# marcinmiklitz/pywindow

Hardware: AMD Instinct MI355X
Metric: trajectory frames/sec full_analysis (pore+windows), CC3 1k-frame (higher is better)
Workload: dtype f64

## Files before the change

pywindow_amd/csrc/pw_unit.hpp:

```cpp
#pragma once
#include "../../include/pywindow_amd.h"
#include "pw_lbfgsb.hpp"
#include "pw_math.hpp"
#include "pw_team.hpp"
#include <string.h>

#if defined(PW_PROFILE) && defined(__HIPCC__)
__shared__ unsigned long long pw_prof_lds[32];
#define PW_PROF_BASE(ws) ((unsigned long long*)pw_prof_lds)
#endif
#if defined(PW_PROFILE) && defined(__HIP_DEVICE_COMPILE__)
#define PW_T0(var) long long var = wall_clock64()
#if defined(PW_ZPROF) && defined(PW_LB_FINE)
#define PW_T1(ws, slot, var) do { (void)var; } while (0)
#elif defined(PW_BARRIER_PROF)
#define PW_T1(ws, slot, var) do { (void)var; if (T::lane() == 0) { unsigned long long w_ = 0; \
        for (int k_ = 0; k_ < T::NWAVES; ++k_) w_ += atomicExch(&pw_bar_acc[k_], 0ull); \
        atomicAdd(&pw_prof_lds[slot], w_); } } while (0)
#else
#define PW_T1(ws, slot, var) do { if (T::lane() == 0) atomicAdd(&pw_prof_lds[slot], (unsigned long long)(wall_clock64() - var)); } while (0)
#endif
#else
#define PW_T0(var) do {} while (0)
#define PW_T1(ws, slot, var) do {} while (0)
#endif

namespace pw {

constexpr double GOLDEN_ANGLE = 2.399963229728653;
constexpr double FOUR_PI = 12.566370614359172;
constexpr double FOUR_THIRDS_PI = 4.1887902047863905;
constexpr double TWO_PI = 6.283185307179586;
constexpr double ONE_PI = 3.141592653589793;

constexpr int PW_KCLS = 8;
constexpr double PW_PATH_POINTS_MAX = 1048576.0;
struct ClassInfo {
    int k;
    int off[PW_KCLS + 1];
    double vdw[PW_KCLS];
};
struct Frame {
    ldouble *x, *y, *z, *xx;
    const ldouble* vdw;
    const lint* perm;
    const PW_LDS ClassInfo* cls;
};

struct TeamWorkspace {
    double* knn;
    double* pts;
    double* vals;
    int* surv_k;
    int* labels;
    unsigned char* flag;
    unsigned long long* adj;
    double* xw;
    int* xw_ok;
    int p_cap;
    const unsigned* nb_off;
    const unsigned short* nb_idx;
    const double* nb_unit;
    const double* nb_bound;
    pw_extra_window* xwin;
    unsigned* xwin_count;
    unsigned xwin_cap;
    double leaf[256];
    double acc8[8 * 160];
    int leaf_tab[324];
    unsigned long long prof[32];
    const unsigned* rsq;
    pw_unit_debug* dbg_base;
    long unit;
};
PW_HD inline size_t team_slab_bytes(int p_cap) { return (size_t)p_cap * 192; }
PW_HD inline size_t team_adj_words(int p_cap) { return (size_t)p_cap * (size_t)(p_cap / 64); }
PW_HD inline int round_p_cap(long p) {
    if (p < PW_P_MAX) p = PW_P_MAX;
    return (int)((p + 127) & ~127l);
}
PW_HD inline int params_p_cap(double adjust_windows, double adjust_average) {
    double a = adjust_windows > adjust_average ? adjust_windows : adjust_average;
    if (!(a > 0.0)) a = 1.0;
    double want = 2100.0 * a;
    if (want > 4.0e6) want = 4.0e6;
    return round_p_cap((long)want + 1);
}
PW_HD inline void bind_team_slab(TeamWorkspace* ws, unsigned char* slab, int p_cap) {
    const size_t p = (size_t)p_cap;
    double* d = (double*)slab;
    ws->knn = d; d += 10 * p;
    ws->pts = d; d += 3 * p;
    ws->vals = d; d += p;
    ws->xw = d; d += 7 * p;
    int* i = (int*)d;
    ws->surv_k = i; i += p;
    ws->labels = i; i += p;
    ws->xw_ok = i; i += p;
    ws->flag = (unsigned char*)i;
    ws->p_cap = p_cap;
}

struct UnitVars {
    double com[3];
    double mw;
    int mw_given;
    double centroid[3];
    double maxd;
    int maxd_i, maxd_j;
    double pore_g;
    int pore_atom;
    double opt_c[3];
    double opt_g;
    int opt_atom;
    double shift[3];
    ClassInfo cls;
    int cls_cnt[PW_KCLS];
    double eps;
// ... 1329 lines not shown
        k0 += NP;
    };
    while (k0 <= chunks && ok) {
        if (chunks - k0 + 1 <= 5) tile(std::integral_constant<int, 5>());
        else tile(std::integral_constant<int, 6>());
    }
    if (n_eval) *n_eval += chunks + 1;
    if (!ok) return false;
    *out_2gap = best * 2.0;
    *out_pos = pos;
    out_chunk[0] = cx; out_chunk[1] = cy; out_chunk[2] = cz;
    return true;
}

struct PathSteps {
    double cx, cy, cz, cd, rinv;
    int chunks;
    bool bracket;
};
PW_HD inline PathSteps path_steps(const Frame& F, double vx, double vy, double vz, double inc, double xx_max) {
    PathSteps s;
    const double nrm = norm3(vx, vy, vz);
    const double fd = np_floordiv(nrm, inc);
    s.bracket = F.cls->k > 0 && fd >= 1.0 && fd <= PW_PATH_POINTS_MAX && nrm < PW_INF;
    s.chunks = s.bracket ? (int)fd : 0;
    s.cd = (double)s.chunks;
    s.cx = vx / s.cd; s.cy = vy / s.cd; s.cz = vz / s.cd;
    const double cc = sq3(s.cx, s.cy, s.cz);
    s.rinv = 1.0 / cc;
    const double bound = (64.0 * 0x1p-53) * (xx_max + sq3(vx, vy, vz));
    s.bracket = s.bracket && cc > 0.0 && cc < PW_INF && s.rinv < PW_INF && bound < PW_INF && cc * (1.0 - 1e-6) > bound;
    return s;
}
PW_NOINLINE PW_HD inline bool path_bracket_thread(const Frame& F, int n, double cx, double cy, double cz, int chunks,
                                                  double rinv, double m0, double* out_2gap, int* n_eval,
                                                  const lint* cand = nullptr, const lint* coff = nullptr,
                                                  long* n_terms = nullptr) {
    (void)n;
    const auto& C = *F.cls;
    const double cd = (double)chunks;
    double best = PW_INF;
    long terms = 0;
    for (int g = 0; g < C.k; ++g) {
        double m2 = PW_INF;
        auto atom = [&](double x, double y, double z, double xx) __attribute__((always_inline)) {
            const double t = pw_fma(z, cz, pw_fma(x, cx, y * cy)) * rinv;
            const double lo = __builtin_fmin(__builtin_fmax(__builtin_floor(t), 1.0), cd);
            const double hi = __builtin_fmin(lo + 1.0, cd);
            const double ax = cx * lo, ay = cy * lo, az = cz * lo;
            const double bx = cx * hi, by = cy * hi, bz = cz * hi;
            const double ga = pw_fma(z, az, pw_fma(x, ax, y * ay));
            const double gb = pw_fma(z, bz, pw_fma(x, bx, y * by));
            const double va = pw_m2add(ga, xx) + sq3(ax, ay, az);
            const double vb = pw_m2add(gb, xx) + sq3(bx, by, bz);
            m2 = __builtin_fmin(m2, __builtin_fmin(va, vb));
        };
        auto span = [&](int c, const int chi, auto at) __attribute__((always_inline)) {
            terms += 2 * (chi - c);
            for (; c + 4 <= chi; c += 4) {
                int i[4];
                double x[4], y[4], z[4], xx[4];
#pragma unroll
                for (int j = 0; j < 4; ++j) i[j] = at(c + j);
#pragma unroll
                for (int j = 0; j < 4; ++j) { x[j] = F.x[i[j]]; y[j] = F.y[i[j]]; z[j] = F.z[i[j]]; xx[j] = F.xx[i[j]]; }
#pragma unroll
                for (int j = 0; j < 4; ++j) atom(x[j], y[j], z[j], xx[j]);
            }
            for (; c < chi; ++c) {
                const int i = at(c);
                atom(F.x[i], F.y[i], F.z[i], F.xx[i]);
            }
        };
        if (cand) span(coff[g], coff[g + 1], [&](int c) __attribute__((always_inline)) { return (int)cand[c]; });
        else span(C.off[g], C.off[g + 1], [](int c) __attribute__((always_inline)) { return c; });
        const double d = pw_sqrt(m2 > 0.0 ? m2 : 0.0);
        best = __builtin_fmin(best, d - C.vdw[g]);
    }
    if (n_eval) *n_eval += chunks + 1;
    if (n_terms) *n_terms += terms;
    if (!(m0 > 0.0) || !(best > 0.0)) return false;
    *out_2gap = (best < m0 ? best : m0) * 2.0;
    return true;
}

template <class T>
PW_HD inline bool wave_path_candidates(const Frame& F, int n, bool have, double vx, double vy, double vz, double inc,
                                       double m0, lint* cand, lint* coff) {
    const auto& C = *F.cls;
    if (C.k == 0 || !(m0 > 0.0)) return false;
    double uz_lo = PW_INF, uz_hi = -PW_INF, t1 = PW_INF;
    bool odd = false;
    if (have) {
        const double nrm = norm3(vx, vy, vz);
        odd = !(nrm >= inc * (1.0 + 1e-9)) || !(nrm < PW_INF) || !(inc > 0.0);
        if (!odd) uz_lo = uz_hi = vz / nrm;
    }
    if (T::wave_any(odd)) return false;
    double z1 = T::wave_min(uz_lo) - 1e-9, z2 = -T::wave_min(-uz_hi) + 1e-9;
    t1 = inc * (1.0 - 1e-9);
    if (!(z1 <= z2)) return false;
    z1 = pw_max(z1, -1.0); z2 = pw_min(z2, 1.0);
    const double s1 = pw_sqrt(pw_max(1.0 - z1 * z1, 0.0)), s2 = pw_sqrt(pw_max(1.0 - z2 * z2, 0.0));
    const double m0p = m0 * (1.0 + 1e-9) + 1e-9;
    const int mycut = T::lane() <= C.k ? C.off[T::lane() <= PW_KCLS ? T::lane() : PW_KCLS] : n;
    int mycount = 0, cnt = 0;
    for (int base = 0; base < n; base += T::WSIZE) {
        const int i = base + T::lane();
        bool keep = false;
        if (i < n) {
            const double xx = F.xx[i], z = F.z[i], r = F.vdw[i];
            const double rho = pw_sqrt(xx);
            const double zd = rho > 0.0 ? z / rho : 0.0;
            const double sd = pw_sqrt(pw_max(1.0 - zd * zd, 0.0));
            double c1 = 1.0;
            if (zd > z2) c1 = sd * s2 + zd * z2;
            else if (zd < z1) c1 = sd * s1 + zd * z1;
            c1 = pw_min(1.0, pw_max(0.0, c1 + 1e-9));
            const double ts = rho * c1;
            const double low = ts >= t1 ? xx * (1.0 - c1 * c1) : (xx + t1 * t1) - 2.0 * t1 * ts;
            const double lim = (r + m0p) * (r + m0p);
            keep = !(low * (1.0 - 1e-9) - 1e-9 > lim * (1.0 + 1e-9));
        }
        const unsigned long long bal = T::ballot(keep);
        const int pos = cnt + __builtin_popcountll(bal & ((1ull << T::lane()) - 1ull));
        if (keep) cand[pos] = i;
        if (T::WSIZE > 1) {
            int w = mycut - base;
            w = w < 0 ? 0 : (w > 64 ? 64 : w);
            mycount += __builtin_popcountll(bal & (w >= 64 ? ~0ull : ((1ull << w) - 1ull)));
        }
        cnt += __builtin_popcountll(bal);
    }
    if (T::WSIZE > 1) {
        if (T::lane() <= C.k) coff[T::lane()] = mycount;
    } else {
        int c = 0;
        for (int g = 0; g <= C.k; ++g) {
            while (c < cnt && cand[c] < C.off[g]) ++c;
            coff[g] = c;
        }
    }
    T::wave_sync();
    return true;
}

PW_HD inline size_t template_groups_bytes(int n) {
    const size_t npad = (size_t)((n + 1) & ~1);
    return ((sizeof(ClassInfo) + 7) & ~(size_t)7) + npad * 4 * 2 + npad * 8 + 8;
}
PW_HD inline double molecular_weight_sum(const double* mass, int n) {
    double tot = 0.0;
    for (int s0 = 0; s0 < n; s0 += 8192) {
        double part = np_sum_lean(mass + s0, n - s0 < 8192 ? n - s0 : 8192);
        tot = s0 == 0 ? part : tot + part;
    }
    return tot;
}
inline void template_groups_build(const double* vdw, const double* mass, int n, unsigned char* blob) {
    const size_t npad = (size_t)((n + 1) & ~1);
    ClassInfo* cls = (ClassInfo*)blob;
    int* inv = (int*)(blob + ((sizeof(ClassInfo) + 7) & ~(size_t)7));
    int* perm = inv + npad;
    double* vs = (double*)(perm + npad);
    memset(blob, 0, template_groups_bytes(n));
    int ngrp = 0;
// ... 1034 lines not shown
#pragma unroll
        for (int g = 0; g <= PW_KCLS; ++g) {
            const int first = g < kk ? T::uniform_i(C->off[g]) : n;
            const int below = first - 64 * t;
            const unsigned long long lt = below >= 64 ? ~0ull : (below <= 0 ? 0ull : ((1ull << below) - 1ull));
            coff[g] += (int)__builtin_popcountll(mk & lt);
        }
        total += (int)__builtin_popcountll(mk);
    }
    if (total > cap || total == 0) return false;
    T::wave_sync();
    double qx[7], qy[7], pp[7], ub[7];
#pragma unroll
    for (int p = 0; p < 7; ++p) {
        int q = lane + 64 * p;
        if (q >= 400) q = lane;
        qx[p] = (double)(q / 20) * gstep + gstart;
        qy[p] = (double)(q % 20) * gstep + gstart;
        pp[p] = sq3(qx[p], qy[p], zopt);
        ub[p] = PW_INF;
    }
#pragma unroll
    for (int g = 0; g < PW_KCLS; ++g) {
        if (g >= kk) continue;
        double m2[7];
#pragma unroll
        for (int p = 0; p < 7; ++p) m2[p] = PW_INF;
        const int jlo = coff[g], jhi = coff[g + 1];
        for (int j = jlo; j < jhi; ++j) {
            const double x = sx[j], y = sy[j], z = sz[j], xx = sq[j];
#pragma unroll
            for (int p = 0; p < 7; ++p) {
                const double gg = pw_fma(z, zopt, pw_fma(x, qx[p], y * qy[p]));
                m2[p] = __builtin_fmin(m2[p], pw_m2add(gg, xx));
            }
        }
        const double r = C->vdw[g];
#pragma unroll
        for (int p = 0; p < 7; ++p) {
            const double m2p = m2[p] + pp[p];
            const double d = pw_sqrt(m2p > 0.0 ? m2p : 0.0);
            ub[p] = __builtin_fmin(ub[p], d - r);
        }
    }
    double ubest = -PW_INF;
    int uq = 0x7fffffff;
#pragma unroll
    for (int p = 0; p < 7; ++p) {
        const int q = lane + 64 * p;
        if (q < 400 && ub[p] > ubest) { ubest = ub[p]; uq = q; }
    }
    {
        double neg = -ubest;
        T::wave_argmin(neg, uq);
        ubest = -neg;
    }
    if (!(ubest < PW_INF) || uq >= 400) return false;
    double best = wave_gap_value<T>(R, n, (double)(uq / 20) * gstep + gstart, (double)(uq % 20) * gstep + gstart, zopt);
    int bestq = uq;
    int left = 0;
    unsigned long long sv[7];
#pragma unroll
    for (int p = 0; p < 7; ++p) {
        const int q = lane + 64 * p;
        sv[p] = T::ballot(q < 400 && q != uq && ub[p] >= best);
        left += (int)__builtin_popcountll(sv[p]);
    }
    if (left > 24) return false;
#pragma unroll
    for (int p = 0; p < 7; ++p) {
        unsigned long long mk = sv[p];
        while (mk) {
            const int q = (int)__builtin_ctzll(mk) + 64 * p;
            mk &= mk - 1ull;
            const double m = wave_gap_value<T>(R, n, (double)(q / 20) * gstep + gstart, (double)(q % 20) * gstep + gstart, zopt);
            if (m > best || (m == best && q < bestq)) { best = m; bestq = q; }
        }
    }
    *gidx_out = bestq;
    return true;
}
#endif

#if defined(__HIP_DEVICE_COMPILE__)
template <class T>
PW_NOINLINE __device__ inline bool wave_path_tube(Frame F, int n, PW_LDS double* scratch, int cap, double cx, double cy,
                                                  double cz, int chunks, double* pbest_out, int* ppos_out, bool* ok_out) {
    const PW_LDS ClassInfo* C = F.cls;
    const int kk = T::uniform_i(C->k);
    cap = T::uniform_i(cap);
    n = T::uniform_i(n);
    chunks = T::uniform_i(chunks);
    if (kk == 0 || cap < 16 || n > 256 || chunks < 16) return false;
    PW_LDS double *sx = scratch, *sy = scratch + cap, *sz = scratch + 2 * cap, *sq = scratch + 3 * cap;
    const int lane = T::lane();
    double T0;
    {
        double px[4], py[4], pz[4], gv[4];
#pragma unroll
        for (int q = 0; q < 4; ++q) {
            const int k = (int)(((long)chunks * (4 + q)) / 8);
            px[q] = cx * (double)k; py[q] = cy * (double)k; pz[q] = cz * (double)k;
        }
        wave_gap4<T>(F, n, px, py, pz, gv);
        T0 = __builtin_fmin(__builtin_fmin(gv[0], gv[1]), __builtin_fmin(gv[2], gv[3]));
    }
    if (!(pw_abs(T0) < 1.0e6)) return false;
    const double ex = cx * (double)chunks, ey = cy * (double)chunks, ez = cz * (double)chunks;
    const double len2 = sq3(ex, ey, ez);
    if (!(len2 > 0.0) || !(len2 < 1.0e12)) return false;
    int coff[PW_KCLS + 1];
#pragma unroll
    for (int g = 0; g <= PW_KCLS; ++g) coff[g] = 0;
    int total = 0;
#pragma unroll
    for (int t = 0; t < 4; ++t) {
        if (64 * t >= n) continue;
        const int i = lane + 64 * t;
        const int ic = i < n ? i : 0;
        const double ax = F.x[ic], ay = F.y[ic], az = F.z[ic], aq = F.xx[ic];
        double s = (ax * ex + ay * ey + az * ez) / len2;
        s = s < 0.0 ? 0.0 : (s > 1.0 ? 1.0 : s);
        const double dx = ax - s * ex, dy = ay - s * ey, dz = az - s * ez;
        const double d2 = dx * dx + dy * dy + dz * dz;
        const double lim = T0 + F.vdw[ic] + 1e-6;
        const bool in = i < n && lim >= 0.0 && d2 <= lim * lim * (1.0 + 1e-9);
        const unsigned long long mk = T::ballot(in);
        const int at = total + (int)__builtin_popcountll(mk & ((1ull << lane) - 1ull));
        if (in && at < cap) { sx[at] = ax; sy[at] = ay; sz[at] = az; sq[at] = aq; }
#pragma unroll
        for (int g = 0; g <= PW_KCLS; ++g) {
            const int first = g < kk ? T::uniform_i(C->off[g]) : n;
            const int below = first - 64 * t;
            const unsigned long long lt = below >= 64 ? ~0ull : (below <= 0 ? 0ull : ((1ull << below) - 1ull));
            coff[g] += (int)__builtin_popcountll(mk & lt);
        }
        total += (int)__builtin_popcountll(mk);
    }
    if (total > cap || total == 0) return false;
    T::wave_sync();
    double pbest = PW_INF;
    int ppos = 0x7fffffff;
    bool ok = true;
    for (int k0 = lane; k0 <= chunks; k0 += 128) {
        const int k1 = k0 + 64 <= chunks ? k0 + 64 : k0;
        const double qx[2] = {cx * (double)k0, cx * (double)k1};
        const double qy[2] = {cy * (double)k0, cy * (double)k1};
        const double qz[2] = {cz * (double)k0, cz * (double)k1};
        double best[2] = {PW_INF, PW_INF};
        const double pp[2] = {sq3(qx[0], qy[0], qz[0]), sq3(qx[1], qy[1], qz[1])};
#pragma unroll
        for (int g = 0; g < PW_KCLS; ++g) {
            if (g >= kk) continue;
            double m2[2] = {PW_INF, PW_INF};
            const int jlo = coff[g], jhi = coff[g + 1];
            int j = jlo;
            for (; j + 4 <= jhi; j += 4) {
                double bx[4], by[4], bz[4], bq[4];
#pragma unroll
                for (int t = 0; t < 4; ++t) { bx[t] = sx[j + t]; by[t] = sy[j + t]; bz[t] = sz[j + t]; bq[t] = sq[j + t]; }
#pragma unroll
                for (int t = 0; t < 4; ++t)
#pragma unroll
                    for (int p = 0; p < 2; ++p) {
                        const double gg = pw_fma(bz[t], qz[p], pw_fma(bx[t], qx[p], by[t] * qy[p]));
                        m2[p] = __builtin_fmin(m2[p], pw_m2add(gg, bq[t]));
                    }
            }
            for (; j < jhi; ++j) {
                const double bx = sx[j], by = sy[j], bz = sz[j], bq = sq[j];
#pragma unroll
                for (int p = 0; p < 2; ++p) {
                    const double gg = pw_fma(bz, qz[p], pw_fma(bx, qx[p], by * qy[p]));
                    m2[p] = __builtin_fmin(m2[p], pw_m2add(gg, bq));
                }
            }
            const double r = C->vdw[g];
#pragma unroll
            for (int p = 0; p < 2; ++p) {
                const double m2p = m2[p] + pp[p];
                const double d = pw_sqrt(m2p > 0.0 ? m2p : 0.0);
                best[p] = __builtin_fmin(best[p], d - r);
            }
        }
        if (!(best[0] > 0.0)) ok = false;
        if (best[0] < pbest) { pbest = best[0]; ppos = k0; }
        if (k1 != k0) {
            if (!(best[1] > 0.0)) ok = false;
            if (best[1] < pbest) { pbest = best[1]; ppos = k1; }
        }
    }
    T::wave_sync();
    *pbest_out = pbest;
    *ppos_out = ppos;
    *ok_out = ok;
    return true;
}
#endif

struct WinArrays {
    double* vec;
    double* d;
    double* c;
    int* ok;
};
template <class T>
PW_NOINLINE PW_HD inline void wave_window(const Frame& FS, const Frame& R, PW_LDS void* lbmem, TeamWorkspace* ws, int n,
                                          int cluster, const double* shift, const pw_params& prm, const WinArrays& wa,
                                          int* evals_sink) {
    int evals = 0;
    double vx = wa.vec[3 * cluster], vy = wa.vec[3 * cluster + 1], vz = wa.vec[3 * cluster + 2];
    PW_T0(t_p);
    double nrm = norm3(vx, vy, vz);
    int chunks = (int)np_floordiv(nrm, prm.increment2);
    double cx = vx / (double)chunks, cy = vy / (double)chunks, cz = vz / (double)chunks;
    double pbest = PW_INF;
    int ppos = 0x7fffffff;
    bool ok = true;
    bool tubed = false;
#if defined(__HIP_DEVICE_COMPILE__)
    if (T::WSIZE == 64)
        tubed = wave_path_tube<T>(FS, n, (PW_LDS double*)lbmem, (int)(sizeof(LbMem<1>) / 8 / 4), cx, cy, cz, chunks, &pbest, &ppos, &ok);
#endif
    if (tubed) {
    } else if (T::WSIZE == 64) {
        for (int k0 = T::lane(); k0 <= chunks; k0 += 2 * T::WSIZE) {
            int k1 = k0 + T::WSIZE <= chunks ? k0 + T::WSIZE : k0;
            double qx[2] = {cx * (double)k0, cx * (double)k1};
            double qy[2] = {cy * (double)k0, cy * (double)k1};
            double qz[2] = {cz * (double)k0, cz * (double)k1};
            double m[2];
            points_gap_values<2>(FS, n, qx, qy, qz, m);
            if (!(m[0] > 0.0)) ok = false;
            if (m[0] < pbest) { pbest = m[0]; ppos = k0; }
            if (k1 != k0) {
                if (!(m[1] > 0.0)) ok = false;
                if (m[1] < pbest) { pbest = m[1]; ppos = k1; }
            }
        }
    } else {
        for (int k = T::lane(); k <= chunks; k += T::WSIZE) {
            double m = point_gap_value(FS, n, cx * (double)k, cy * (double)k, cz * (double)k);
            if (!(m > 0.0)) ok = false;
            if (m < pbest) { pbest = m; ppos = k; }
        }
    }
    evals += chunks + 1;
    ok = T::wave_all(ok);
    if (!ok) {
        if (T::lane() == 0) {
            wa.ok[cluster] = 0;
            *evals_sink += evals;
        }
        return;
    }
    T::wave_argmin(pbest, ppos);
    PW_T1(ws, 2, t_p);
    PW_T0(t_r);
    double new_z = norm3(cx * (double)ppos, cy * (double)ppos, cz * (double)ppos);
    double vx2, vy2, vz2;
    if (T::WSIZE == 64) {
        const double sq = pw_square_np(T::lane() == 1 ? vy : (T::lane() == 2 ? vz : vx));
        vx2 = T::bcast_u(sq, 0); vy2 = T::bcast_u(sq, 1); vz2 = T::bcast_u(sq, 2);
    } else {
        vx2 = pw_square_np(vx); vy2 = pw_square_np(vy); vz2 = pw_square_np(vz);
    }
    double c1 = pw_abs(vx * 1.0 + vy * 0.0 + 0.0 * 0.0) /
                (pw_sqrt(vx2 + vy2 + 0.0) * pw_sqrt(1.0 + 0.0 + 0.0));
    double c2 = pw_abs(vx * 0.0 + vy * 0.0 + vz * 1.0) /
                (pw_sqrt(vx2 + vy2 + vz2) * pw_sqrt(0.0 + 0.0 + 1.0));
    double a1, a2;
    if (T::WSIZE == 64) {
        const double ac = pw_acos_np(T::lane() == 1 ? c2 : c1, ws->rsq);
        a1 = T::bcast_u(ac, 0); a2 = T::bcast_u(ac, 1);
    } else {
        a1 = pw_acos_np(c1, ws->rsq); a2 = pw_acos_np(c2, ws->rsq);
    }
    const double a1_raw = a1, a2_raw = a2;
    bool sxp = vx >= 0.0, syp = vy >= 0.0, szp = vz >= 0.0;
    if (szp) {
        if (sxp && syp) { a1 = -a1; a2 = -a2; }
        else if (!sxp && syp) { a1 = TWO_PI + a1; }
        else if (sxp && !syp) { a2 = -a2; }
        else { a1 = TWO_PI - a1; }
    } else {
        if (sxp && syp) { a1 = -a1; a2 = ONE_PI + a2; }
        else if (!sxp && syp) { a2 = ONE_PI - a2; }
        else if (sxp && !syp) { a2 = a2 + ONE_PI; }
        else { a1 = -a1; a2 = ONE_PI - a2; }
    }
    double s1, co1, s2, co2;
    if (T::WSIZE == 64) {
        double sv, cv;
        pw_sincos(T::lane() == 1 ? a2 : a1, &sv, &cv);
        s1 = T::bcast_u(sv, 0); co1 = T::bcast_u(cv, 0); s2 = T::bcast_u(sv, 1); co2 = T::bcast_u(cv, 1);
    } else {
        pw_sincos(a1, &s1, &co1);
        pw_sincos(a2, &s2, &co2);
    }
    auto row = [](double m0, double m1, double m2, double x, double y, double z) {
        return pw_fma(m2, z, pw_fma(m0, x, m1 * y));
    };
    for (int i = T::lane(); i < n; i += T::WSIZE) {
        double x = FS.x[i], y = FS.y[i], z = FS.z[i];
        double x1 = row(co1, -s1, 0.0, x, y, z);
        double y1 = row(s1, co1, 0.0, x, y, z);
        double z1 = row(0.0, 0.0, 1.0, x, y, z);
        double x2 = row(co2, 0.0, s2, x1, y1, z1);
        double y2 = row(0.0, 1.0, 0.0, x1, y1, z1);
        double z2 = row(-s2, 0.0, co2, x1, y1, z1);
        x2 = x2 - 0.0; y2 = y2 - 0.0; z2 = z2 - new_z;
        R.x[i] = x2; R.y[i] = y2; R.z[i] = z2;
        R.xx[i] = sq3(x2, y2, z2);
    }
    T::wave_sync();
    double d0 = wave_gap_value<T>(R, n, 0.0, 0.0, 0.0) * 2.0;
    evals += 1;
    PW_T1(ws, 3, t_r);
    Lbfgsb<1> zopt_state;
    Lbfgsb<1>* S = &zopt_state;
    LbMem<1>* Smem = (LbMem<1>*)lbmem;
    PW_ASSUME_LDS(Smem);
    double lo1[1] = {prm.lb_z ? -new_z : prm.z_lo}, up1[1] = {prm.z_hi};
    int nbd1[1];
    {
        bool has_lo = lo1[0] > -PW_INF, has_up = up1[0] < PW_INF;
        nbd1[0] = has_lo ? (has_up ? 2 : 1) : (has_up ? 3 : 0);
    }
    if (lo1[0] > up1[0]) {
        if (T::lane() == 0) {
            wa.ok[cluster] = -1;
            *evals_sink += evals;
        }
        return;
    }
    double xo = 0.0, yo = 0.0, zopt = 0.0;
    for (int phase = 0; phase < 2; ++phase) {
        if (lo1[0] == up1[0]) {
            zopt = lo1[0];
// ... 561 lines not shown
        }
        double m = sum / (double)(P * 10);
        if (T::tid() == 0) { v.eps = m + pw_pow_np(m, 0.5); out->eps = v.eps; }
        T::sync();
        if (T::wave() == 0) PW_T1(ws, 25, t_sum);
    }
    if (T::wave() == 0) PW_T1(ws, 8, t_eps);
    PW_T0(t_smp);
    arena = arena_pts;
    double* vals = (double*)arena.take((size_t)P * 8);
    if (!vals) vals = ws->vals;
    int* surv_k = (int*)arena.take((size_t)P * 4);
    if (!surv_k) surv_k = ws->surv_k;
    int* labels = (int*)arena.take((size_t)P * 4);
    if (!labels) labels = ws->labels;
    unsigned char* flag = (unsigned char*)arena.take((size_t)P);
    if (!flag) flag = ws->flag;
    ScratchArena arena_mark = arena;
    double* tmpv = (double*)arena.take((size_t)P * 8);
    if (!tmpv) tmpv = ws->knn;
    {
        double cen[3] = {v.centroid[0], v.centroid[1], v.centroid[2]};
        bool done = false;
        {
            for (int k = T::tid(); k < P; k += T::SIZE) flag[k] = 1;
            ScratchArena a2 = arena_mark;
            ConeBand* bands = (ConeBand*)a2.take((size_t)n * sizeof(ConeBand));
            ConeLattice* lat = bands ? take_cone_lattice(a2, n) : nullptr;
            int cap = (int)(a2.left / 4);
            unsigned* pairs = (unsigned*)a2.take((size_t)cap * 4);
            if (cap < 4 * P) { pairs = (unsigned*)ws->knn; cap = 16 * ws->p_cap; }
            if (!bands && (size_t)n * sizeof(ConeBand) <= (size_t)ws->p_cap * 16) bands = (ConeBand*)(ws->knn + 8 * (size_t)ws->p_cap);
            auto run = [&](auto pts_) __attribute__((always_inline)) {
                SpiralRays<decltype(pts_)> getp{pts_, Q4};
                return team_ray_tests<T, false>(sh.S, n, cen, sp, getp, bands, pairs, cap, (PW_LDS int*)&v.red_i[0], flag, 0, nullptr, lat);
            };
            if (bands) done = PW_IS_LDS(pts) ? run(PW_AS_LDS(pts)) : run(pts);
        }
        if (done) {
        } else if (T::SIZE > 1) {
            constexpr int NR = 4;
            for (int k0 = T::tid(); k0 < P; k0 += NR * T::SIZE) {
                double dx[NR], dy[NR], dz[NR], far[NR];
                bool hit[NR];
#pragma unroll
                for (int r = 0; r < NR; ++r) {
                    int k = k0 + r * T::SIZE < P ? k0 + r * T::SIZE : k0;
                    dx[r] = pts[PT(k, 0)]; dy[r] = pts[PT(k, 1)]; dz[r] = pts[PT(k, 2)];
                }
                ray_scan_multi<NR, false>(sh.S, n, cen, dx, dy, dz, hit, far);
#pragma unroll
                for (int r = 0; r < NR; ++r) {
                    int k = k0 + r * T::SIZE;
                    if (k < P) flag[k] = hit[r] ? 0 : 1;
                }
            }
        } else {
            for (int k = T::tid(); k < P; k += T::SIZE) {
                double far;
                bool hit = ray_scan(sh.S, n, cen, pts[PT(k, 0)], pts[PT(k, 1)], pts[PT(k, 2)], &far);
                flag[k] = hit ? 0 : 1;
            }
        }
        T::sync();
        if (T::wave() == 0) {
            int m = 0;
            for (int base = 0; base < P; base += T::WSIZE) {
                int k = base + T::lane();
                bool f = k < P && flag[k] != 0;
                unsigned long long bal = T::ballot(f);
                int pos = m + __builtin_popcountll(bal & ((1ull << T::lane()) - 1ull));
                if (f) labels[pos] = k;
                m += __builtin_popcountll(bal);
            }
            if (T::lane() == 0) v.n_surv = m;
        }
        T::sync();
        int ncand = v.n_surv;
        int evals = 0;
        if (T::wave() == 0) PW_T1(ws, 30, t_smp);
        PW_T0(t_path);
        const double m_origin = wave_gap_value<T>(sh.S, n, 0.0, 0.0, 0.0);
        int whole = T::SIZE > 1 ? (ncand / T::SIZE) * T::SIZE : ncand;
        if ((ncand - whole) * 16 >= T::SIZE) whole = ncand;
        lint* cand_w = nullptr;
        lint* coff_w = nullptr;
        {
            ScratchArena a3 = arena;
            const size_t per_wave = (size_t)n + PW_KCLS + 2;
            int* c_all = (int*)a3.take((size_t)T::NWAVES * per_wave * 4);
#ifndef PW_NO_SCAN_LISTS
            if (c_all && PW_IS_LDS(c_all)) {
                cand_w = (lint*)PW_AS_LDS(c_all) + (size_t)T::wave() * per_wave;
                coff_w = cand_w + n;
            }
#endif
        }
#ifndef PW_NO_PATH_BRACKETS
        double xx_max = 0.0;
        if (whole > 0) {
            for (int i = T::lane(); i < n; i += T::WSIZE) xx_max = __builtin_fmax(xx_max, sh.S.xx[i]);
            xx_max = -T::wave_min(-xx_max);
        }
#endif
        for (int j0 = 0; j0 < whole; j0 += T::SIZE) {
            const int j = j0 + T::tid();
            const bool have = j < whole;
            const int k = have ? labels[j] : 0;
            const double vx = pts[PT(k, 0)], vy = pts[PT(k, 1)], vz = pts[PT(k, 2)];
            const bool listed = cand_w != nullptr &&
                                wave_path_candidates<T>(sh.S, n, have, vx, vy, vz, prm.increment, m_origin, cand_w, coff_w);
#ifndef PW_NO_PATH_BRACKETS
            const PathSteps steps = path_steps(sh.S, vx, vy, vz, prm.increment, xx_max);
            if (!T::wave_any(have && !steps.bracket)) {
                if (have) {
                    double g2 = 0.0;
                    bool ok = path_bracket_thread(sh.S, n, steps.cx, steps.cy, steps.cz, steps.chunks, steps.rinv, m_origin,
                                                  &g2, &evals, listed ? cand_w : nullptr, listed ? coff_w : nullptr);
                    flag[j] = ok ? 1 : 0;
                    tmpv[j] = g2;
                }
                continue;
            }
#endif
            if (have) {
                double g2, chunk[3];
                int pos;
                bool ok = path_scan_thread(sh.S, n, vx, vy, vz, prm.increment, m_origin, &g2, &pos, chunk, &evals,
                                           listed ? cand_w : nullptr, listed ? coff_w : nullptr);
                flag[j] = ok ? 1 : 0;
                tmpv[j] = g2;
            }
        }
        const int left = ncand - whole;
        if (left > 0) {
            for (int j = whole + T::wave(); j < ncand; j += T::NWAVES) {
                const int k = labels[j];
                const double vx = pts[PT(k, 0)], vy = pts[PT(k, 1)], vz = pts[PT(k, 2)];
                const int chunks = (int)np_floordiv(norm3(vx, vy, vz), prm.increment);
                double g2 = 0.0;
                bool ok = true;
                bool all_at_once = false;
                if constexpr (T::WSIZE == 64) all_at_once = chunks >= 1 && chunks <= 16 && sh.S.cls->k > 0;
                if (all_at_once) {
                    if constexpr (T::WSIZE == 64) {
                        const auto& C = *sh.S.cls;
                        const Frame& F = sh.S;
                        const double cx = vx / (double)chunks, cy = vy / (double)chunks, cz = vz / (double)chunks;
                        const int sub = T::lane() & 3;
                        const int q = (T::lane() >> 2) + 1 <= chunks ? (T::lane() >> 2) + 1 : chunks;
                        const double qx = cx * (double)q, qy = cy * (double)q, qz = cz * (double)q;
                        const double pp = sq3(qx, qy, qz);
                        double gap = PW_INF;
                        for (int g = 0; g < C.k; ++g) {
                            double m2 = PW_INF;
                            const int hi = C.off[g + 1];
                            for (int i = C.off[g] + sub; i < hi; i += 4) {
                                const double x = F.x[i], y = F.y[i], z = F.z[i], xx = F.xx[i];
                                const double gg = pw_fma(z, qz, pw_fma(x, qx, y * qy));
                                m2 = __builtin_fmin(m2, pw_m2add(gg, xx));
                            }
                            m2 = __builtin_fmin(m2, T::xor_d(m2, 1));
                            m2 = __builtin_fmin(m2, T::xor_d(m2, 2));
                            const double m2p = m2 + pp;
                            const double d = pw_sqrt(m2p > 0.0 ? m2p : 0.0);
                            gap = __builtin_fmin(gap, d - C.vdw[g]);
                        }
                        double best = m_origin;
                        if (!(m_origin > 0.0)) ok = false;
                        for (int q2 = 1; q2 <= chunks && ok; ++q2) {
                            const double m = T::bcast_u(gap, 4 * (q2 - 1));
                            if (!(m > 0.0)) ok = false;
                            else if (m < best) best = m;
                        }
                        g2 = best * 2.0;
                    }
                } else if (chunks >= 1) {
                    const double cx = vx / (double)chunks, cy = vy / (double)chunks, cz = vz / (double)chunks;
                    double best = m_origin;
                    if (!(m_origin > 0.0)) ok = false;
                    for (int q = 1; q <= chunks && ok; ++q) {
                        const double m = wave_gap_value<T>(sh.S, n, cx * (double)q, cy * (double)q, cz * (double)q);
                        if (!(m > 0.0)) ok = false;
                        else if (m < best) best = m;
                    }
                    g2 = best * 2.0;
                } else {
                    double chunk[3];
                    int pos;
                    ok = path_scan_thread(sh.S, n, vx, vy, vz, prm.increment, m_origin, &g2, &pos, chunk, &evals);
                }
                if (T::lane() == 0) { flag[j] = ok ? 1 : 0; tmpv[j] = g2; }
            }
        }
        T::sync();
        if (T::wave() == 0) PW_T1(ws, 31, t_path);
        if (T::wave() == 0) {
            int m = 0;
            for (int base = 0; base < ncand; base += T::WSIZE) {
                int j = base + T::lane();
                bool f = j < ncand && flag[j] != 0;
                unsigned long long bal = T::ballot(f);
                int pos = m + __builtin_popcountll(bal & ((1ull << T::lane()) - 1ull));
                if (f) { surv_k[pos] = labels[j]; vals[pos] = tmpv[j]; }
                m += __builtin_popcountll(bal);
            }
            if (T::lane() == 0) { v.n_surv = m; out->n_survivors = m; }
        }
        T::sync();
        (void)evals;
    }
    if (T::wave() == 0) PW_T1(ws, 9, t_smp);
    int ns = v.n_surv;
    if (ns == 0) {
        if (T::tid() == 0) out->n_windows = -1;
        T::sync();
        return -1;
    }
    PW_T0(t_db);
    arena = arena_mark;
    {
        const int label = team_dbscan<T>(sh.bits[0], sh.bits[1], sh.bits[2], arena, ws, pts, PT, surv_k, ns, v.eps, labels);
        if (label < 0) {
            if (T::tid() == 0) v.status |= PW_ST_POINTS_OVERFLOW;
            T::sync();
            return -1;
        }
        if (T::tid() == 0) {
            v.n_clusters = label;
            out->n_clusters = label;
        }
        if (label > PW_W_MAX) {
            wa.vec = ws->xw; wa.d = ws->xw + 3 * (size_t)ws->p_cap; wa.c = ws->xw + 4 * (size_t)ws->p_cap; wa.ok = ws->xw_ok;
        }
        for (int c = T::tid(); c < label; c += T::SIZE) wa.ok[c] = 0;
        T::sync();
        for (int c = T::wave(); c < label; c += T::NWAVES) {
            double best = -PW_INF;
            int bidx = 0x7fffffff;
            for (int q = T::lane(); q < ns; q += T::WSIZE) {
                if (labels[q] == c) {
                    double val = vals[q];
                    if (val > best || (val == best && q < bidx)) { best = val; bidx = q; }
                }
            }
            T::wave_argmax(best, bidx);
            if (T::lane() == 0) {
                const int pvk = surv_k[bidx];
                wa.vec[3 * c] = pts[PT(pvk, 0)]; wa.vec[3 * c + 1] = pts[PT(pvk, 1)]; wa.vec[3 * c + 2] = pts[PT(pvk, 2)];
            }
        }
        T::sync();
        if (pw_unit_debug* dbg = ws->dbg_base ? ws->dbg_base + ws->unit : nullptr) {
            for (int i = T::tid(); i < ns && i < PW_P_MAX; i += T::SIZE) {
                dbg->pass_idx[i] = surv_k[i];
                dbg->labels[i] = labels[i];
                dbg->gap2[i] = vals[i];
            }
            if (T::tid() == 0) { dbg->n_survivors = ns; dbg->n_clusters = label; }
// ... 156 lines not shown
```

Before: 1.042 million.

## Replace path tube scan with per-atom bracket minimum along window paths

Adds wave_path_bracket, which projects each atom onto the path direction and evaluates only the two neighbouring sampled chunk points, so the minimum gap is found in O(atoms) instead of O(atoms×chunks). It replaces the LDS-based tube filter in the window path refinement and the all-at-once small-chunk path in the leftover candidate loop, when path_steps reports that a bracket is valid. It also makes the leftover rounding threshold a macro and computes xx_max whenever there are candidates. This relies on the per-atom distance along the line being unimodal, so that the bracket holds the true minimum. It also changes the tie-breaking and fallback behaviour.

```diff
diff --git a/pywindow_amd/csrc/pw_unit.hpp b/pywindow_amd/csrc/pw_unit.hpp
--- a/pywindow_amd/csrc/pw_unit.hpp
+++ b/pywindow_amd/csrc/pw_unit.hpp
@@ -34,6 +34,9 @@
 constexpr double ONE_PI = 3.141592653589793;
 
 constexpr int PW_KCLS = 8;
+#ifndef PW_LEFTOVER_ROUND_DIV
+#define PW_LEFTOVER_ROUND_DIV 16
+#endif
 constexpr double PW_PATH_POINTS_MAX = 1048576.0;
 struct ClassInfo {
     int k;
@@ -1529,6 +1532,44 @@
     if (!(m0 > 0.0) || !(best > 0.0)) return false;
     *out_2gap = (best < m0 ? best : m0) * 2.0;
     return true;
+}
+
+struct PathMin {
+    double gap;
+    int k;
+};
+template <class T>
+PW_NOINLINE PW_HD inline PathMin wave_path_bracket(const Frame& F, int n, double cx, double cy, double cz, int chunks,
+                                                   double rinv, int k_first, long* n_terms = nullptr) {
+    const double kf = (double)k_first, cd = (double)chunks;
+    double best = PW_INF;
+    int pos = 0x7fffffff;
+    long terms = 0;
+    for (int i = T::lane(); i < n; i += T::WSIZE) {
+        const double x = F.x[i], y = F.y[i], z = F.z[i], xx = F.xx[i], r = F.vdw[i];
+        const double t = pw_fma(z, cz, pw_fma(x, cx, y * cy)) * rinv;
+        const double lo = __builtin_fmin(__builtin_fmax(__builtin_floor(t), kf), cd);
+        const double hi = __builtin_fmin(lo + 1.0, cd);
+        const double ax = cx * lo, ay = cy * lo, az = cz * lo;
+        const double bx = cx * hi, by = cy * hi, bz = cz * hi;
+        const double ga = pw_fma(z, az, pw_fma(x, ax, y * ay));
+        const double gb = pw_fma(z, bz, pw_fma(x, bx, y * by));
+        const double va = pw_m2add(ga, xx) + sq3(ax, ay, az);
+        const double vb = pw_m2add(gb, xx) + sq3(bx, by, bz);
+        const double da = pw_sqrt(va > 0.0 ? va : 0.0) - r;
+        const double db = pw_sqrt(vb > 0.0 ? vb : 0.0) - r;
+        const int ka = (int)lo, kb = (int)hi;
+        if (da < best || (da == best && ka < pos)) { best = da; pos = ka; }
+        if (db < best || (db == best && kb < pos)) { best = db; pos = kb; }
+        terms += 2;
+    }
+    T::wave_argmin(best, pos);
+    if (!(best < PW_INF)) pos = 0x7fffffff;
+    if (n_terms) *n_terms += terms;
+    PathMin out;
+    out.gap = best;
+    out.k = pos;
+    return out;
 }
 
 template <class T>
@@ -2729,122 +2770,6 @@
 }
 #endif
 
-#if defined(__HIP_DEVICE_COMPILE__)
-template <class T>
-PW_NOINLINE __device__ inline bool wave_path_tube(Frame F, int n, PW_LDS double* scratch, int cap, double cx, double cy,
-                                                  double cz, int chunks, double* pbest_out, int* ppos_out, bool* ok_out) {
-    const PW_LDS ClassInfo* C = F.cls;
-    const int kk = T::uniform_i(C->k);
-    cap = T::uniform_i(cap);
-    n = T::uniform_i(n);
-    chunks = T::uniform_i(chunks);
-    if (kk == 0 || cap < 16 || n > 256 || chunks < 16) return false;
-    PW_LDS double *sx = scratch, *sy = scratch + cap, *sz = scratch + 2 * cap, *sq = scratch + 3 * cap;
-    const int lane = T::lane();
-    double T0;
-    {
-        double px[4], py[4], pz[4], gv[4];
-#pragma unroll
-        for (int q = 0; q < 4; ++q) {
-            const int k = (int)(((long)chunks * (4 + q)) / 8);
-            px[q] = cx * (double)k; py[q] = cy * (double)k; pz[q] = cz * (double)k;
-        }
-        wave_gap4<T>(F, n, px, py, pz, gv);
-        T0 = __builtin_fmin(__builtin_fmin(gv[0], gv[1]), __builtin_fmin(gv[2], gv[3]));
-    }
-    if (!(pw_abs(T0) < 1.0e6)) return false;
-    const double ex = cx * (double)chunks, ey = cy * (double)chunks, ez = cz * (double)chunks;
-    const double len2 = sq3(ex, ey, ez);
-    if (!(len2 > 0.0) || !(len2 < 1.0e12)) return false;
-    int coff[PW_KCLS + 1];
-#pragma unroll
-    for (int g = 0; g <= PW_KCLS; ++g) coff[g] = 0;
-    int total = 0;
-#pragma unroll
-    for (int t = 0; t < 4; ++t) {
-        if (64 * t >= n) continue;
-        const int i = lane + 64 * t;
-        const int ic = i < n ? i : 0;
-        const double ax = F.x[ic], ay = F.y[ic], az = F.z[ic], aq = F.xx[ic];
-        double s = (ax * ex + ay * ey + az * ez) / len2;
-        s = s < 0.0 ? 0.0 : (s > 1.0 ? 1.0 : s);
-        const double dx = ax - s * ex, dy = ay - s * ey, dz = az - s * ez;
-        const double d2 = dx * dx + dy * dy + dz * dz;
-        const double lim = T0 + F.vdw[ic] + 1e-6;
-        const bool in = i < n && lim >= 0.0 && d2 <= lim * lim * (1.0 + 1e-9);
-        const unsigned long long mk = T::ballot(in);
-        const int at = total + (int)__builtin_popcountll(mk & ((1ull << lane) - 1ull));
-        if (in && at < cap) { sx[at] = ax; sy[at] = ay; sz[at] = az; sq[at] = aq; }
-#pragma unroll
-        for (int g = 0; g <= PW_KCLS; ++g) {
-            const int first = g < kk ? T::uniform_i(C->off[g]) : n;
-            const int below = first - 64 * t;
-            const unsigned long long lt = below >= 64 ? ~0ull : (below <= 0 ? 0ull : ((1ull << below) - 1ull));
-            coff[g] += (int)__builtin_popcountll(mk & lt);
-        }
-        total += (int)__builtin_popcountll(mk);
-    }
-    if (total > cap || total == 0) return false;
-    T::wave_sync();
-    double pbest = PW_INF;
-    int ppos = 0x7fffffff;
-    bool ok = true;
-    for (int k0 = lane; k0 <= chunks; k0 += 128) {
-        const int k1 = k0 + 64 <= chunks ? k0 + 64 : k0;
-        const double qx[2] = {cx * (double)k0, cx * (double)k1};
-        const double qy[2] = {cy * (double)k0, cy * (double)k1};
-        const double qz[2] = {cz * (double)k0, cz * (double)k1};
-        double best[2] = {PW_INF, PW_INF};
-        const double pp[2] = {sq3(qx[0], qy[0], qz[0]), sq3(qx[1], qy[1], qz[1])};
-#pragma unroll
-        for (int g = 0; g < PW_KCLS; ++g) {
-            if (g >= kk) continue;
-            double m2[2] = {PW_INF, PW_INF};
-            const int jlo = coff[g], jhi = coff[g + 1];
-            int j = jlo;
-            for (; j + 4 <= jhi; j += 4) {
-                double bx[4], by[4], bz[4], bq[4];
-#pragma unroll
-                for (int t = 0; t < 4; ++t) { bx[t] = sx[j + t]; by[t] = sy[j + t]; bz[t] = sz[j + t]; bq[t] = sq[j + t]; }
-#pragma unroll
-                for (int t = 0; t < 4; ++t)
-#pragma unroll
-                    for (int p = 0; p < 2; ++p) {
-                        const double gg = pw_fma(bz[t], qz[p], pw_fma(bx[t], qx[p], by[t] * qy[p]));
-                        m2[p] = __builtin_fmin(m2[p], pw_m2add(gg, bq[t]));
-                    }
-            }
-            for (; j < jhi; ++j) {
-                const double bx = sx[j], by = sy[j], bz = sz[j], bq = sq[j];
-#pragma unroll
-                for (int p = 0; p < 2; ++p) {
-                    const double gg = pw_fma(bz, qz[p], pw_fma(bx, qx[p], by * qy[p]));
-                    m2[p] = __builtin_fmin(m2[p], pw_m2add(gg, bq));
-                }
-            }
-            const double r = C->vdw[g];
-#pragma unroll
-            for (int p = 0; p < 2; ++p) {
-                const double m2p = m2[p] + pp[p];
-                const double d = pw_sqrt(m2p > 0.0 ? m2p : 0.0);
-                best[p] = __builtin_fmin(best[p], d - r);
-            }
-        }
-        if (!(best[0] > 0.0)) ok = false;
-        if (best[0] < pbest) { pbest = best[0]; ppos = k0; }
-        if (k1 != k0) {
-            if (!(best[1] > 0.0)) ok = false;
-            if (best[1] < pbest) { pbest = best[1]; ppos = k1; }
-        }
-    }
-    T::wave_sync();
-    *pbest_out = pbest;
-    *ppos_out = ppos;
-    *ok_out = ok;
-    return true;
-}
-#endif
-
 struct WinArrays {
     double* vec;
     double* d;
@@ -2864,12 +2789,23 @@
     double pbest = PW_INF;
     int ppos = 0x7fffffff;
     bool ok = true;
-    bool tubed = false;
-#if defined(__HIP_DEVICE_COMPILE__)
-    if (T::WSIZE == 64)
-        tubed = wave_path_tube<T>(FS, n, (PW_LDS double*)lbmem, (int)(sizeof(LbMem<1>) / 8 / 4), cx, cy, cz, chunks, &pbest, &ppos, &ok);
-#endif
-    if (tubed) {
+    bool bracketed = false;
+#ifndef PW_NO_PATH_BRACKETS
+    {
+        double xx_max = 0.0;
+        for (int i = T::lane(); i < n; i += T::WSIZE) xx_max = __builtin_fmax(xx_max, FS.xx[i]);
+        xx_max = -T::wave_min(-xx_max);
+        const PathSteps steps = path_steps(FS, vx, vy, vz, prm.increment2, xx_max);
+        if (steps.bracket && steps.chunks == chunks && steps.cx == cx && steps.cy == cy && steps.cz == cz) {
+            const PathMin pm = wave_path_bracket<T>(FS, n, cx, cy, cz, chunks, steps.rinv, 0);
+            pbest = pm.gap;
+            ppos = pm.k;
+            ok = pm.gap > 0.0;
+            bracketed = true;
+        }
+    }
+#endif
+    if (bracketed) {
     } else if (T::WSIZE == 64) {
         for (int k0 = T::lane(); k0 <= chunks; k0 += 2 * T::WSIZE) {
             int k1 = k0 + T::WSIZE <= chunks ? k0 + T::WSIZE : k0;
@@ -2901,7 +2837,7 @@
         }
         return;
     }
-    T::wave_argmin(pbest, ppos);
+    if (!bracketed) T::wave_argmin(pbest, ppos);
     PW_T1(ws, 2, t_p);
     PW_T0(t_r);
     double new_z = norm3(cx * (double)ppos, cy * (double)ppos, cz * (double)ppos);
@@ -3629,7 +3565,7 @@
         PW_T0(t_path);
         const double m_origin = wave_gap_value<T>(sh.S, n, 0.0, 0.0, 0.0);
         int whole = T::SIZE > 1 ? (ncand / T::SIZE) * T::SIZE : ncand;
-        if ((ncand - whole) * 16 >= T::SIZE) whole = ncand;
+        if ((ncand - whole) * PW_LEFTOVER_ROUND_DIV >= T::SIZE) whole = ncand;
         lint* cand_w = nullptr;
         lint* coff_w = nullptr;
         {
@@ -3645,7 +3581,7 @@
         }
 #ifndef PW_NO_PATH_BRACKETS
         double xx_max = 0.0;
-        if (whole > 0) {
+        if (ncand > 0) {
             for (int i = T::lane(); i < n; i += T::WSIZE) xx_max = __builtin_fmax(xx_max, sh.S.xx[i]);
             xx_max = -T::wave_min(-xx_max);
         }
@@ -3687,41 +3623,19 @@
                 const int chunks = (int)np_floordiv(norm3(vx, vy, vz), prm.increment);
                 double g2 = 0.0;
                 bool ok = true;
-                bool all_at_once = false;
-                if constexpr (T::WSIZE == 64) all_at_once = chunks >= 1 && chunks <= 16 && sh.S.cls->k > 0;
-                if (all_at_once) {
-                    if constexpr (T::WSIZE == 64) {
-                        const auto& C = *sh.S.cls;
-                        const Frame& F = sh.S;
-                        const double cx = vx / (double)chunks, cy = vy / (double)chunks, cz = vz / (double)chunks;
-                        const int sub = T::lane() & 3;
-                        const int q = (T::lane() >> 2) + 1 <= chunks ? (T::lane() >> 2) + 1 : chunks;
-                        const double qx = cx * (double)q, qy = cy * (double)q, qz = cz * (double)q;
-                        const double pp = sq3(qx, qy, qz);
-                        double gap = PW_INF;
-                        for (int g = 0; g < C.k; ++g) {
-                            double m2 = PW_INF;
-                            const int hi = C.off[g + 1];
-                            for (int i = C.off[g] + sub; i < hi; i += 4) {
-                                const double x = F.x[i], y = F.y[i], z = F.z[i], xx = F.xx[i];
-                                const double gg = pw_fma(z, qz, pw_fma(x, qx, y * qy));
-                                m2 = __builtin_fmin(m2, pw_m2add(gg, xx));
-                            }
-                            m2 = __builtin_fmin(m2, T::xor_d(m2, 1));
-                            m2 = __builtin_fmin(m2, T::xor_d(m2, 2));
-                            const double m2p = m2 + pp;
-                            const double d = pw_sqrt(m2p > 0.0 ? m2p : 0.0);
-                            gap = __builtin_fmin(gap, d - C.vdw[g]);
-                        }
-                        double best = m_origin;
-                        if (!(m_origin > 0.0)) ok = false;
-                        for (int q2 = 1; q2 <= chunks && ok; ++q2) {
-                            const double m = T::bcast_u(gap, 4 * (q2 - 1));
-                            if (!(m > 0.0)) ok = false;
-                            else if (m < best) best = m;
-                        }
-                        g2 = best * 2.0;
+                bool bracketed = false;
+#ifndef PW_NO_PATH_BRACKETS
+                {
+                    const PathSteps steps = path_steps(sh.S, vx, vy, vz, prm.increment, xx_max);
+                    if (steps.bracket) {
+                        const PathMin pm = wave_path_bracket<T>(sh.S, n, steps.cx, steps.cy, steps.cz, steps.chunks, steps.rinv, 1);
+                        ok = m_origin > 0.0 && pm.gap > 0.0;
+                        if (ok) g2 = (pm.gap < m_origin ? pm.gap : m_origin) * 2.0;
+                        bracketed = true;
                     }
+                }
+#endif
+                if (bracketed) {
                 } else if (chunks >= 1) {
                     const double cx = vx / (double)chunks, cy = vy / (double)chunks, cz = vz / (double)chunks;
                     double best = m_origin;
```

After: 1.066 million (median of 6 runs). +2.3%, better.
